# FangjinhuaWang/PatchmatchNet

Measured on AMD Instinct MI355X. Metric: depth-maps/sec at 1600x1200 N=5 src views, higher is better.
Workload: dtype f32

## Files before the change

patchmatchnet_amd/csrc/conv_f16s.hip:

```cpp
#include "pmn_common.hpp"

typedef _Float16 f16x8 __attribute__((ext_vector_type(8)));
typedef _Float16 f16x4 __attribute__((ext_vector_type(4)));
typedef float f32x4_t __attribute__((ext_vector_type(4)));
typedef float f32x2_t __attribute__((ext_vector_type(2)));
typedef _Float16 f16x2_t __attribute__((ext_vector_type(2)));

struct F16sArgs {
    int N, H, W, Ho, Wo, relu;
    int cout, ca;
    float* out_b;
};

#define PMN_F16S_LO_SCALE 2048.0f

template <int CIN, int COUT, int KS, int S, int CC, int CCP, int MT, int WPS, int DIL = 1, int OUTMODE = 0, bool SWAP = (OUTMODE == 0)>
__global__ __launch_bounds__(256, WPS) void conv_f16s_kernel(const float* __restrict__ in, const f16x8* __restrict__ wB,
                                                             const float* __restrict__ shift, float* __restrict__ out,
                                                             const F16sArgs a) {
    constexpr int NT = COUT / 16, NCB = CC / 8, CHUNKS = CIN / CC, NQ = KS * KS * NCB, KSTEPS = (NQ + 3) / 4;
    constexpr int TH = 4 * MT, TW = 16, PH = (TH - 1) * S + (KS - 1) * DIL + 1, PW = (TW - 1) * S + (KS - 1) * DIL + 1;
    constexpr int PAD = DIL * (KS / 2);
    constexpr int PLANE = PH * PW * CCP;
    constexpr int NTHR = 256;
    static_assert(!SWAP || OUTMODE == 0, "swapped operand roles (see the epilogue) serve the channels-last output");
    static_assert(CCP % 8 == 0 && CC % 8 == 0 && CIN % CC == 0, "16-byte aligned channel blocks");
    extern __shared__ float4 f16s_lds4[];
    _Float16* Phi = reinterpret_cast<_Float16*>(f16s_lds4);
    _Float16* Plo = Phi + PLANE;
    const int tid = threadIdx.x, wave = __builtin_amdgcn_readfirstlane(tid >> 6), lane = tid & 63, li = lane & 15, kb = lane >> 4;
    const int tiles_x = (a.Wo + TW - 1) / TW, tiles_y = (a.Ho + TH - 1) / TH;
    const int bt = pmn_xcd_tile(blockIdx.x, a.N * tiles_x * tiles_y);
    const int n = bt / (tiles_x * tiles_y), tr = bt - n * tiles_x * tiles_y;
    const int oy0 = (tr / tiles_x) * TH, ox0 = (tr % tiles_x) * TW;
    const int iy0 = oy0 * S - PAD, ix0 = ox0 * S - PAD;

    f32x4_t accM[MT][NT], accL[MT][NT];
#pragma unroll
    for (int t = 0; t < MT; ++t)
#pragma unroll
        for (int nt = 0; nt < NT; ++nt) {
            accM[t][nt] = f32x4_t{0.f, 0.f, 0.f, 0.f};
            accL[t][nt] = f32x4_t{0.f, 0.f, 0.f, 0.f};
        }

    const f16x8* bl = wB + lane;
    f16x8 bq[2][NT][2];
#pragma unroll
    for (int nt = 0; nt < NT; ++nt) {
        bq[0][nt][0] = bl[(size_t)((0 * NT + nt) * 2 + 0) * 64];
        bq[0][nt][1] = bl[(size_t)((0 * NT + nt) * 2 + 1) * 64];
    }

    const int q4x4 = 4 * (tid % (CC / 4)), pix_first = tid / (CC / 4);
    const int py_first = pix_first / PW, px_first = pix_first - py_first * PW, lds_first = pix_first * CCP + q4x4;

#pragma unroll 1
    for (int ch = 0; ch < CHUNKS; ++ch) {
        if (ch) __syncthreads();
        {
            constexpr int QP = CC / 4, TOT = PH * PW * QP, NL = (TOT + NTHR - 1) / NTHR, SB = 6;
            constexpr int DPIX = NTHR / QP, DY = DPIX / PW, DX = DPIX - DY * PW;
            static_assert(NTHR % QP == 0, "a step of NTHR units is a whole number of pixels");
            const float* src = in + (size_t)n * a.H * a.W * CIN + ch * CC;
            int py = py_first, px = px_first;
#pragma unroll
            for (int k0 = 0; k0 < NL; k0 += SB) {
                float4 v[SB];
#pragma unroll
                for (int k = 0; k < SB; ++k) {
                    const int gy = iy0 + py, gx = ix0 + px;
                    v[k] = make_float4(0.f, 0.f, 0.f, 0.f);
                    if (k0 + k < NL && tid < TOT - (k0 + k) * NTHR && (unsigned)gy < (unsigned)a.H && (unsigned)gx < (unsigned)a.W)
                        v[k] = *reinterpret_cast<const float4*>(src + ((unsigned)(gy * a.W + gx) * CIN + q4x4));
                    px += DX;
                    py += DY;
                    if (px >= PW) {
                        px -= PW;
                        ++py;
                    }
                }
#pragma unroll
                for (int k = 0; k < SB; ++k) {
                    if (k0 + k < NL && tid < TOT - (k0 + k) * NTHR) {
                        const f32x2_t x01 = {v[k].x, v[k].y}, x23 = {v[k].z, v[k].w};
                        const f16x2_t h01 = __builtin_convertvector(x01, f16x2_t), h23 = __builtin_convertvector(x23, f16x2_t);
                        const f16x2_t l01 = __builtin_convertvector((x01 - __builtin_convertvector(h01, f32x2_t)) * PMN_F16S_LO_SCALE, f16x2_t);
                        const f16x2_t l23 = __builtin_convertvector((x23 - __builtin_convertvector(h23, f32x2_t)) * PMN_F16S_LO_SCALE, f16x2_t);
                        const f16x4 hi = {h01[0], h01[1], h23[0], h23[1]}, lo = {l01[0], l01[1], l23[0], l23[1]};
                        *reinterpret_cast<f16x4*>(Phi + lds_first + (k0 + k) * DPIX * CCP) = hi;
                        *reinterpret_cast<f16x4*>(Plo + lds_first + (k0 + k) * DPIX * CCP) = lo;
                    }
                }
            }
        }
        __syncthreads();

#pragma unroll
        for (int ks = 0; ks < KSTEPS; ++ks) {
            constexpr int dummy = 0;
            (void)dummy;
            const int cur = ks & 1, nxt = cur ^ 1;
            {
                const int step = ch * KSTEPS + ks + 1;
                const int lim = CHUNKS * KSTEPS - 1;
                const int sidx = step < lim ? step : lim;
#pragma unroll
                for (int nt = 0; nt < NT; ++nt) {
                    bq[nxt][nt][0] = bl[(size_t)((sidx * NT + nt) * 2 + 0) * 64];
                    bq[nxt][nt][1] = bl[(size_t)((sidx * NT + nt) * 2 + 1) * 64];
                }
            }
            int q = 4 * ks + kb;
            if (4 * ks + 3 >= NQ) q = q < NQ - 1 ? q : NQ - 1;
            const int tap = q / NCB, cb = q - tap * NCB;
            const int dy = tap / KS, dx = tap - dy * KS;
            const _Float16* pa = Phi + ((wave * MT * S + dy * DIL) * PW + li * S + dx * DIL) * CCP + cb * 8;
            f16x8 ah[MT], al[MT];
#pragma unroll
            for (int t = 0; t < MT; ++t) {
                ah[t] = *reinterpret_cast<const f16x8*>(pa + t * S * PW * CCP);
                al[t] = *reinterpret_cast<const f16x8*>(pa + t * S * PW * CCP + PLANE);
            }
#pragma unroll
            for (int t = 0; t < MT; ++t)
#pragma unroll
                for (int nt = 0; nt < NT; ++nt)
                    accM[t][nt] = SWAP ? __builtin_amdgcn_mfma_f32_16x16x32_f16(bq[cur][nt][0], ah[t], accM[t][nt], 0, 0, 0)
                                       : __builtin_amdgcn_mfma_f32_16x16x32_f16(ah[t], bq[cur][nt][0], accM[t][nt], 0, 0, 0);
#pragma unroll
            for (int t = 0; t < MT; ++t)
#pragma unroll
                for (int nt = 0; nt < NT; ++nt)
                    accL[t][nt] = SWAP ? __builtin_amdgcn_mfma_f32_16x16x32_f16(bq[cur][nt][1], ah[t], accL[t][nt], 0, 0, 0)
                                       : __builtin_amdgcn_mfma_f32_16x16x32_f16(ah[t], bq[cur][nt][1], accL[t][nt], 0, 0, 0);
#pragma unroll
            for (int t = 0; t < MT; ++t)
#pragma unroll
                for (int nt = 0; nt < NT; ++nt)
                    accL[t][nt] = SWAP ? __builtin_amdgcn_mfma_f32_16x16x32_f16(bq[cur][nt][0], al[t], accL[t][nt], 0, 0, 0)
                                       : __builtin_amdgcn_mfma_f32_16x16x32_f16(al[t], bq[cur][nt][0], accL[t][nt], 0, 0, 0);
            __builtin_amdgcn_sched_barrier(0);
        }
        if (KSTEPS & 1) {
#pragma unroll
            for (int nt = 0; nt < NT; ++nt) {
                bq[0][nt][0] = bq[1][nt][0];
                bq[0][nt][1] = bq[1][nt][1];
            }
        }
    }

    if constexpr (SWAP) {
        const int ox = ox0 + li, oyw = oy0 + wave * MT;
        if (ox < a.Wo) {
            float* po = out + (((size_t)n * a.Ho + oyw) * a.Wo + ox) * COUT + 4 * kb;
            const size_t rs = (size_t)a.Wo * COUT;
            f32x4_t sh[NT];
#pragma unroll
            for (int nt = 0; nt < NT; ++nt) sh[nt] = *reinterpret_cast<const f32x4_t*>(shift + 16 * nt + 4 * kb);
#pragma unroll
            for (int t = 0; t < MT; ++t) {
                if (oyw + t < a.Ho) {
#pragma unroll
                    for (int nt = 0; nt < NT; ++nt) {
                        f32x4_t v = accM[t][nt] + accL[t][nt] * (1.0f / PMN_F16S_LO_SCALE) + sh[nt];
                        if (a.relu) v = __builtin_elementwise_max(v, f32x4_t{0.f, 0.f, 0.f, 0.f});
                        *reinterpret_cast<f32x4_t*>(po + t * rs + 16 * nt) = v;
                    }
                }
            }
        }
        return;
    }
#pragma unroll
    for (int nt = 0; nt < NT; ++nt) {
        const int c = nt * 16 + li;
        const float sh = shift[c];
#pragma unroll
        for (int t = 0; t < MT; ++t) {
            const int oy = oy0 + wave * MT + t;
            float v[4];
#pragma unroll
            for (int r = 0; r < 4; ++r) {
                v[r] = accM[t][nt][r] + accL[t][nt][r] * (1.0f / PMN_F16S_LO_SCALE) + sh;
                if (a.relu) v[r] = fmaxf(v[r], 0.0f);
            }
            if constexpr (OUTMODE == 0) {
#pragma unroll
                for (int r = 0; r < 4; ++r) {
                    const int ox = ox0 + 4 * kb + r;
                    if (oy < a.Ho && ox < a.Wo) out[(((size_t)n * a.Ho + oy) * a.Wo + ox) * COUT + c] = v[r];
                }
            } else {
                if (c < a.cout && oy < a.Ho) {
                    const bool first = c < a.ca;
                    float* dst = first ? out : a.out_b;
                    const int cx = first ? c : c - a.ca, nc = first ? a.ca : a.cout - a.ca;
                    if constexpr (OUTMODE == 1) {
                        float* row = dst + (((size_t)n * nc + cx) * a.Ho + oy) * a.Wo;
                        const int ox = ox0 + 4 * kb;
                        if ((a.Wo & 3) == 0 && ox + 3 < a.Wo) {
                            *reinterpret_cast<float4*>(row + ox) = make_float4(v[0], v[1], v[2], v[3]);
                        } else {
#pragma unroll
                            for (int r = 0; r < 4; ++r)
                                if (ox + r < a.Wo) row[ox + r] = v[r];
                        }
                    } else {
#pragma unroll
                        for (int r = 0; r < 4; ++r) {
                            const int ox = ox0 + 4 * kb + r;
                            if (ox < a.Wo) dst[(((size_t)n * a.Ho + oy) * a.Wo + ox) * nc + cx] = v[r];
                        }
                    }
                }
            }
        }
    }
}

template <int CIN, int COUT, int KS, int S, int CC, int CCP, int MT, int WPS, int DIL = 1, int OUTMODE = 0, bool SWAP = (OUTMODE == 0)>
static int launch_f16s(const float* in, const void* w, const float* shift, float* out, F16sArgs a, hipStream_t st) {
    constexpr int TH = 4 * MT, PH = (TH - 1) * S + (KS - 1) * DIL + 1, PW = 15 * S + (KS - 1) * DIL + 1;
    const size_t lds = (size_t)2 * PH * PW * CCP * sizeof(_Float16);
    auto kern = conv_f16s_kernel<CIN, COUT, KS, S, CC, CCP, MT, WPS, DIL, OUTMODE, SWAP>;
    if ((size_t)a.H * a.W * CIN >= ((size_t)1 << 30)) return PMN_ERR_SHAPE;
    if (lds > 48 * 1024 && pmn_raise_dynamic_lds(reinterpret_cast<const void*>(kern), lds) != PMN_OK) return PMN_ERR_LAUNCH;
    const int blocks = a.N * ((a.Wo + 15) / 16) * ((a.Ho + TH - 1) / TH);
    PMN_LAUNCH(kern, dim3(blocks), dim3(256), lds, st, in, reinterpret_cast<const f16x8*>(w), shift, out, a);
    PMN_CHECK_LAUNCH();
    return PMN_OK;
}

extern "C" int pmn_conv2d_f16s(const float* in, const void* weights, const float* shift, float* out, int N, int H, int W, int cin,
                               int cout, int k, int stride, int relu, void* stream) {
    if (!in || !weights || !shift || !out || N < 1 || H < 1 || W < 1) return PMN_ERR_ARG;
    F16sArgs a;
    a.N = N; a.H = H; a.W = W; a.relu = relu;
    a.cout = cout; a.ca = cout; a.out_b = nullptr;
    a.Ho = (H - 1) / (stride > 0 ? stride : 1) + 1;
    a.Wo = (W - 1) / (stride > 0 ? stride : 1) + 1;
    hipStream_t st = (hipStream_t)stream;
    if (k == 3 && stride == 1 && cin == 16 && cout == 16) return launch_f16s<16, 16, 3, 1, 16, 16, 4, 4>(in, weights, shift, out, a, st);
    if (k == 3 && stride == 1 && cin == 32 && cout == 32) return launch_f16s<32, 32, 3, 1, 16, 16, 2, 4, 1, 0, false>(in, weights, shift, out, a, st);
    if (k == 3 && stride == 1 && cin == 64 && cout == 64) return launch_f16s<64, 64, 3, 1, 16, 16, 2, 3>(in, weights, shift, out, a, st);
    if (k == 5 && stride == 2 && cin == 8 && cout == 16) return launch_f16s<8, 16, 5, 2, 8, 8, 2, 4>(in, weights, shift, out, a, st);
    if (k == 5 && stride == 2 && cin == 16 && cout == 32) return launch_f16s<16, 32, 5, 2, 8, 8, 2, 4, 1, 0, false>(in, weights, shift, out, a, st);
    if (k == 5 && stride == 2 && cin == 32 && cout == 64) return launch_f16s<32, 64, 5, 2, 16, 24, 2, 2>(in, weights, shift, out, a, st);
    return PMN_ERR_SHAPE;
}


template <int WPS>
__global__ __launch_bounds__(256, WPS) void conv_f16s_pair16_kernel(const float* __restrict__ in, const f16x8* __restrict__ wA,
                                                                   const float* __restrict__ shiftA, const f16x8* __restrict__ wBq,
                                                                   const float* __restrict__ shiftB, float* __restrict__ out,
                                                                   const F16sArgs a) {
    constexpr int C = 16, CCP = 16, NCB = 2, NQ = 18, KSTEPS = 5, TO = 14, RA = 16, PI = 18;
    constexpr int PLANE = PI * PI * CCP;
    extern __shared__ float4 f16s_pair_lds4[];
    _Float16* Phi = reinterpret_cast<_Float16*>(f16s_pair_lds4);
    _Float16* Plo = Phi + PLANE;
    const int tid = threadIdx.x, wave = __builtin_amdgcn_readfirstlane(tid >> 6), lane = tid & 63, li = lane & 15, kb = lane >> 4;
    const int tiles_x = (a.W + TO - 1) / TO, tiles_y = (a.H + TO - 1) / TO;
    const int bt = pmn_xcd_tile(blockIdx.x, a.N * tiles_x * tiles_y);
    const int n = bt / (tiles_x * tiles_y), tr = bt - n * tiles_x * tiles_y;
    const int oy0 = (tr / tiles_x) * TO, ox0 = (tr % tiles_x) * TO;

    {
        constexpr int QP = C / 4, TOT = PI * PI * QP, NL = (TOT + 255) / 256;
        const float* src = in + (size_t)n * a.H * a.W * C;
        float4 v[NL];
#pragma unroll
        for (int k = 0; k < NL; ++k) {
            const int idx = tid + k * 256, pix = idx / QP, q = idx - pix * QP;
            const int py = pix / PI, px = pix - py * PI, gy = oy0 - 2 + py, gx = ox0 - 2 + px;
            v[k] = make_float4(0.f, 0.f, 0.f, 0.f);
            if (idx < TOT && (unsigned)gy < (unsigned)a.H && (unsigned)gx < (unsigned)a.W)
                v[k] = *reinterpret_cast<const float4*>(src + ((unsigned)(gy * a.W + gx) * C + 4 * q));
        }
#pragma unroll
        for (int k = 0; k < NL; ++k) {
            const int idx = tid + k * 256, pix = idx / QP, q = idx - pix * QP;
            if (idx < TOT) {
                const f32x2_t x01 = {v[k].x, v[k].y}, x23 = {v[k].z, v[k].w};
                const f16x2_t h01 = __builtin_convertvector(x01, f16x2_t), h23 = __builtin_convertvector(x23, f16x2_t);
                const f16x2_t l01 = __builtin_convertvector((x01 - __builtin_convertvector(h01, f32x2_t)) * PMN_F16S_LO_SCALE, f16x2_t);
                const f16x2_t l23 = __builtin_convertvector((x23 - __builtin_convertvector(h23, f32x2_t)) * PMN_F16S_LO_SCALE, f16x2_t);
                const f16x4 hi = {h01[0], h01[1], h23[0], h23[1]}, lo = {l01[0], l01[1], l23[0], l23[1]};
                *reinterpret_cast<f16x4*>(Phi + pix * CCP + 4 * q) = hi;
                *reinterpret_cast<f16x4*>(Plo + pix * CCP + 4 * q) = lo;
            }
        }
    }
    __syncthreads();

    f32x4_t accM[4], accL[4];
    auto layer = [&](const f16x8* __restrict__ wq, const int pitch) {
        const f16x8* bl = wq + lane;
        f16x8 bq[2][2];
        bq[0][0] = bl[0];
        bq[0][1] = bl[64];
#pragma unroll
        for (int t = 0; t < 4; ++t) {
            accM[t] = f32x4_t{0.f, 0.f, 0.f, 0.f};
            accL[t] = f32x4_t{0.f, 0.f, 0.f, 0.f};
        }
#pragma unroll
        for (int ks = 0; ks < KSTEPS; ++ks) {
            const int cur = ks & 1, nxt = cur ^ 1;
            const int sidx = ks + 1 < KSTEPS ? ks + 1 : KSTEPS - 1;
            bq[nxt][0] = bl[(size_t)(sidx * 2 + 0) * 64];
            bq[nxt][1] = bl[(size_t)(sidx * 2 + 1) * 64];
            int q = 4 * ks + kb;
            if (4 * ks + 3 >= NQ) q = q < NQ - 1 ? q : NQ - 1;
            const int tap = q / NCB, cb = q - tap * NCB;
            const int dy = tap / 3, dx = tap - dy * 3;
            const _Float16* pa = Phi + ((wave * 4 + dy) * pitch + li + dx) * CCP + cb * 8;
            f16x8 ah[4], al[4];
#pragma unroll
            for (int t = 0; t < 4; ++t) {
                ah[t] = *reinterpret_cast<const f16x8*>(pa + t * pitch * CCP);
                al[t] = *reinterpret_cast<const f16x8*>(pa + t * pitch * CCP + PLANE);
            }
#pragma unroll
            for (int t = 0; t < 4; ++t) accM[t] = __builtin_amdgcn_mfma_f32_16x16x32_f16(bq[cur][0], ah[t], accM[t], 0, 0, 0);
#pragma unroll
            for (int t = 0; t < 4; ++t) accL[t] = __builtin_amdgcn_mfma_f32_16x16x32_f16(bq[cur][1], ah[t], accL[t], 0, 0, 0);
#pragma unroll
            for (int t = 0; t < 4; ++t) accL[t] = __builtin_amdgcn_mfma_f32_16x16x32_f16(bq[cur][0], al[t], accL[t], 0, 0, 0);
            __builtin_amdgcn_sched_barrier(0);
        }
    };

    layer(wA, PI);
    f16x4 rh[4], rl[4];
    {
        const f32x4_t sh = *reinterpret_cast<const f32x4_t*>(shiftA + 4 * kb);
        const int gx = ox0 - 1 + li;
#pragma unroll
        for (int t = 0; t < 4; ++t) {
            const int gy = oy0 - 1 + wave * 4 + t;
            f32x4_t v = accM[t] + accL[t] * (1.0f / PMN_F16S_LO_SCALE) + sh;
            if (a.relu) v = __builtin_elementwise_max(v, f32x4_t{0.f, 0.f, 0.f, 0.f});
            if (!((unsigned)gy < (unsigned)a.H && (unsigned)gx < (unsigned)a.W)) v = f32x4_t{0.f, 0.f, 0.f, 0.f};
            const f32x2_t x01 = {v[0], v[1]}, x23 = {v[2], v[3]};
            const f16x2_t h01 = __builtin_convertvector(x01, f16x2_t), h23 = __builtin_convertvector(x23, f16x2_t);
            const f16x2_t l01 = __builtin_convertvector((x01 - __builtin_convertvector(h01, f32x2_t)) * PMN_F16S_LO_SCALE, f16x2_t);
            const f16x2_t l23 = __builtin_convertvector((x23 - __builtin_convertvector(h23, f32x2_t)) * PMN_F16S_LO_SCALE, f16x2_t);
            rh[t] = f16x4{h01[0], h01[1], h23[0], h23[1]};
            rl[t] = f16x4{l01[0], l01[1], l23[0], l23[1]};
        }
    }
    __syncthreads();
#pragma unroll
    for (int t = 0; t < 4; ++t) {
        const int pix = (wave * 4 + t) * RA + li;
        *reinterpret_cast<f16x4*>(Phi + pix * CCP + 4 * kb) = rh[t];
        *reinterpret_cast<f16x4*>(Plo + pix * CCP + 4 * kb) = rl[t];
    }
    __syncthreads();

    layer(wBq, RA);
    {
        const int ox = ox0 + li;
        if (li < TO && ox < a.W) {
            const f32x4_t sh = *reinterpret_cast<const f32x4_t*>(shiftB + 4 * kb);
#pragma unroll
            for (int t = 0; t < 4; ++t) {
                const int r = wave * 4 + t, oy = oy0 + r;
                if (r < TO && oy < a.H) {
                    f32x4_t v = accM[t] + accL[t] * (1.0f / PMN_F16S_LO_SCALE) + sh;
                    if (a.relu) v = __builtin_elementwise_max(v, f32x4_t{0.f, 0.f, 0.f, 0.f});
                    *reinterpret_cast<f32x4_t*>(out + (((size_t)n * a.H + oy) * a.W + ox) * C + 4 * kb) = v;
                }
            }
        }
    }
}

extern "C" int pmn_conv2d_f16s_pair(const float* in, const void* weights_a, const float* shift_a, const void* weights_b,
                                    const float* shift_b, float* out, int N, int H, int W, int channels, int relu, void* stream) {
    if (!in || !weights_a || !shift_a || !weights_b || !shift_b || !out || N < 1 || H < 1 || W < 1) return PMN_ERR_ARG;
    if (channels != 16) return PMN_ERR_SHAPE;
    if ((size_t)H * W * 16 >= ((size_t)1 << 30)) return PMN_ERR_SHAPE;
    F16sArgs a;
    a.N = N; a.H = H; a.W = W; a.Ho = H; a.Wo = W; a.relu = relu;
    a.cout = 16; a.ca = 16; a.out_b = nullptr;
    const size_t lds = (size_t)2 * 18 * 18 * 16 * sizeof(_Float16);
    const int blocks = N * ((W + 13) / 14) * ((H + 13) / 14);
    PMN_LAUNCH(conv_f16s_pair16_kernel<4>, dim3(blocks), dim3(256), lds, (hipStream_t)stream, in, reinterpret_cast<const f16x8*>(weights_a),
               shift_a, reinterpret_cast<const f16x8*>(weights_b), shift_b, out, a);
    PMN_CHECK_LAUNCH();
    return PMN_OK;
}


template <int CIN, int DIL, int MT, int WPS>
static int dispatch_heads(const float* in, const void* w, const float* shift, float* out_a, int coutp, F16sArgs a, hipStream_t st) {
    if (coutp == 32) return launch_f16s<CIN, 32, 3, 1, 16, 16, MT, WPS, DIL, 1>(in, w, shift, out_a, a, st);
    if (coutp == 48) return launch_f16s<CIN, 48, 3, 1, 16, 16, MT, WPS, DIL, 1>(in, w, shift, out_a, a, st);
    if (coutp == 64) return launch_f16s<CIN, 64, 3, 1, 16, 16, MT, (WPS > 3 ? 3 : WPS), DIL, 1>(in, w, shift, out_a, a, st);
    return PMN_ERR_SHAPE;
}

extern "C" int pmn_offset_heads_f16s(const float* in, const void* weights, const float* shift, float* out_a, float* out_b, int N, int H,
                                     int W, int cin, int cout, int ca, int dil, void* stream) {
    if (!in || !weights || !shift || !out_a || N < 1 || H < 1 || W < 1 || cout < 1 || ca < 1 || ca > cout) return PMN_ERR_ARG;
    if (ca < cout && !out_b) return PMN_ERR_ARG;
    F16sArgs a;
    a.N = N; a.H = H; a.W = W; a.Ho = H; a.Wo = W; a.relu = 0;
    a.cout = cout; a.ca = ca; a.out_b = out_b;
    const int coutp = (cout + 15) / 16 * 16;
    hipStream_t st = (hipStream_t)stream;
    if (cin == 64 && dil == 2) return dispatch_heads<64, 2, 2, 3>(in, weights, shift, out_a, coutp, a, st);
    if (cin == 32 && dil == 4) return dispatch_heads<32, 4, 2, 4>(in, weights, shift, out_a, coutp, a, st);
    if (cin == 16 && dil == 6) return dispatch_heads<16, 6, 2, 4>(in, weights, shift, out_a, coutp, a, st);
    return PMN_ERR_SHAPE;
}

#ifndef PMN_STEM_TH
#define PMN_STEM_TH 32
#endif
template <bool VEC4, int TH>
__global__ __launch_bounds__(256, 4) void stem_f16s_kernel(const float* __restrict__ img, const float* __restrict__ w0,
                                                          const float* __restrict__ s0, const f16x8* __restrict__ w1A,
                                                          const float* __restrict__ s1, float* __restrict__ out, const int N,
                                                          const int H, const int W, const float* const* __restrict__ img_tab,
                                                          const int BV) {
    constexpr int TS = 16, IW = TH + 4, XS = 24, MW = TS + 2, MRP = 18, MROWS = TH + 2, NTHR = 256;
    static_assert(TH % 16 == 0, "a wave owns TH / 4 rows, four at a time");
    __shared__ float4 xin4[3 * IW * (XS / 4)];
    __shared__ float4 mid4[2 * MROWS * MRP];
    float* xin = reinterpret_cast<float*>(xin4);
    _Float16* midh = reinterpret_cast<_Float16*>(mid4);
    _Float16* midl = midh + MROWS * MRP * 8;
    typedef const float __attribute__((address_space(4))) cfloat;
    const cfloat* cw0 = (const cfloat*)w0;
    const cfloat* cs0 = (const cfloat*)s0;
    const int tid = threadIdx.x, wave = __builtin_amdgcn_readfirstlane(tid >> 6), lane = tid & 63, li = lane & 15, kb = lane >> 4;
    const int tiles_x = (W + TS - 1) / TS, tiles_y = (H + TH - 1) / TH;
    const int bt = pmn_xcd_tile(blockIdx.x, N * tiles_x * tiles_y);
    const int n = bt / (tiles_x * tiles_y), tr = bt - n * tiles_x * tiles_y;
    const int oy0 = (tr / tiles_x) * TH, ox0 = (tr % tiles_x) * TS;
    if (img_tab) img = img_tab[n / BV] + (ptrdiff_t)((n % BV) - n) * 3 * H * W;

    f16x8 wa[3][2];
#pragma unroll
    for (int ks = 0; ks < 3; ++ks) {
        wa[ks][0] = w1A[(ks * 2 + 0) * 64 + lane];
        wa[ks][1] = w1A[(ks * 2 + 1) * 64 + lane];
    }
    if constexpr (VEC4) {
        constexpr int NU = (3 * IW + 31) / 32;
        float4 v[NU];
        const int j = tid & 7, gx = ox0 - 4 + 4 * j;
#pragma unroll
        for (int u = 0; u < NU; ++u) {
            const int R = (tid >> 3) + 32 * u;
            const int c = (R >= IW) + (R >= 2 * IW), r = R - IW * c, gy = oy0 - 2 + r;
            v[u] = make_float4(0.f, 0.f, 0.f, 0.f);
            if (j < 6 && R < 3 * IW && (unsigned)gy < (unsigned)H && (unsigned)gx < (unsigned)W)
                v[u] = *reinterpret_cast<const float4*>(img + (((size_t)n * 3 + c) * H + gy) * W + gx);
        }
#pragma unroll
        for (int u = 0; u < NU; ++u) {
            const int R = (tid >> 3) + 32 * u;
            if (j < 6 && R < 3 * IW) xin4[R * (XS / 4) + j] = v[u];
        }
    } else {
        constexpr int NU = (3 * IW + 7) / 8;
        float v[NU];
        const int q = tid & 31, gx = ox0 - 4 + q;
#pragma unroll
        for (int u = 0; u < NU; ++u) {
            const int R = (tid >> 5) + 8 * u;
            const int c = (R >= IW) + (R >= 2 * IW), r = R - IW * c, gy = oy0 - 2 + r;
            v[u] = 0.0f;
            if (q < XS && R < 3 * IW && (unsigned)gy < (unsigned)H && (unsigned)gx < (unsigned)W)
                v[u] = img[(((size_t)n * 3 + c) * H + gy) * W + gx];
        }
#pragma unroll
        for (int u = 0; u < NU; ++u) {
            const int R = (tid >> 5) + 8 * u;
            if (q < XS && R < 3 * IW) xin[R * XS + q] = v[u];
        }
    }
    __syncthreads();
    for (int m = tid; m < MW * MROWS; m += NTHR) {
        const int r = m / MW, q = m - r * MW;
        const int gy = oy0 - 1 + r, gx = ox0 - 1 + q;
        f16x8 hi = {0, 0, 0, 0, 0, 0, 0, 0}, lo = {0, 0, 0, 0, 0, 0, 0, 0};
        if ((unsigned)gy < (unsigned)H && (unsigned)gx < (unsigned)W) {
            float acc[8];
#pragma unroll
            for (int c = 0; c < 8; ++c) acc[c] = 0.0f;
            const float* xp = xin + r * XS + q + 2;
#pragma unroll 1
            for (int ky = 0; ky < 3; ++ky) {
                const cfloat* wq = cw0 + __builtin_amdgcn_readfirstlane(ky * 72);
#pragma unroll
                for (int kx = 0; kx < 3; ++kx)
#pragma unroll
                    for (int ci = 0; ci < 3; ++ci) {
                        const float v = xp[(ci * IW + ky) * XS + kx];
#pragma unroll
                        for (int c = 0; c < 8; ++c) acc[c] = fmaf(v, wq[(kx * 3 + ci) * 8 + c], acc[c]);
                    }
            }
#pragma unroll
            for (int c = 0; c < 8; c += 2) {
                const f32x2_t x = {fmaxf(acc[c] + cs0[c], 0.0f), fmaxf(acc[c + 1] + cs0[c + 1], 0.0f)};
                const f16x2_t h = __builtin_convertvector(x, f16x2_t);
                const f32x2_t d = (x - __builtin_convertvector(h, f32x2_t)) * PMN_F16S_LO_SCALE;
                const f16x2_t l = __builtin_convertvector(d, f16x2_t);
                hi[c] = h[0];
                hi[c + 1] = h[1];
                lo[c] = l[0];
                lo[c + 1] = l[1];
            }
        }
        *reinterpret_cast<f16x8*>(midh + (r * MRP + q) * 8) = hi;
        *reinterpret_cast<f16x8*>(midl + (r * MRP + q) * 8) = lo;
    }
    __syncthreads();
#pragma unroll 1
    for (int rg = 0; rg < TH / 16; ++rg) {
    const int wrow = wave * (TH / 4) + 4 * rg;
    f32x4_t accM[4], accL[4];
#pragma unroll
    for (int t = 0; t < 4; ++t) {
        accM[t] = f32x4_t{0.f, 0.f, 0.f, 0.f};
        accL[t] = f32x4_t{0.f, 0.f, 0.f, 0.f};
    }
#pragma unroll
    for (int ks = 0; ks < 3; ++ks) {
        int q = 4 * ks + kb;
        q = q < 8 ? q : 8;
        const int dy = q / 3, dx = q - dy * 3;
        const _Float16* pb = midh + ((wrow + dy) * MRP + li + dx) * 8;
        f16x8 bh[4], blo[4];
#pragma unroll
        for (int t = 0; t < 4; ++t) {
            bh[t] = *reinterpret_cast<const f16x8*>(pb + t * MRP * 8);
            blo[t] = *reinterpret_cast<const f16x8*>(pb + t * MRP * 8 + MROWS * MRP * 8);
        }
#pragma unroll
        for (int t = 0; t < 4; ++t) accM[t] = __builtin_amdgcn_mfma_f32_16x16x32_f16(wa[ks][0], bh[t], accM[t], 0, 0, 0);
#pragma unroll
        for (int t = 0; t < 4; ++t) accL[t] = __builtin_amdgcn_mfma_f32_16x16x32_f16(wa[ks][0], blo[t], accL[t], 0, 0, 0);
#pragma unroll
        for (int t = 0; t < 4; ++t) accL[t] = __builtin_amdgcn_mfma_f32_16x16x32_f16(wa[ks][1], bh[t], accL[t], 0, 0, 0);
    }
    const int ox = ox0 + li, oyw = oy0 + wrow;
    if (kb < 2 && ox < W) {
        const f32x4_t sh = *reinterpret_cast<const f32x4_t*>(s1 + 4 * kb);
        float* po = out + (((size_t)n * H + oyw) * W + ox) * 8 + 4 * kb;
        const size_t rs = (size_t)W * 8;
#pragma unroll
        for (int t = 0; t < 4; ++t) {
            if (oyw + t < H) {
                f32x4_t v = accM[t] + accL[t] * (1.0f / PMN_F16S_LO_SCALE) + sh;
                v = __builtin_elementwise_max(v, f32x4_t{0.f, 0.f, 0.f, 0.f});
                *reinterpret_cast<f32x4_t*>(po + t * rs) = v;
            }
        }
    }
    }
}

extern "C" int pmn_stem_f16s(const float* img, const float* w0, const float* s0, const void* w1a, const float* s1, float* out,
                             int N, int H, int W, void* stream) {
    if (!img || !w0 || !s0 || !w1a || !s1 || !out || N < 1 || H < 1 || W < 1) return PMN_ERR_ARG;
    constexpr int TS = 16, TH = PMN_STEM_TH;
    const int blocks = N * ((W + TS - 1) / TS) * ((H + TH - 1) / TH);
    if (W % 4 == 0 && (reinterpret_cast<uintptr_t>(img) & 15) == 0)
        PMN_LAUNCH((stem_f16s_kernel<true, PMN_STEM_TH>), dim3(blocks), dim3(256), 0, (hipStream_t)stream, img, w0, s0,
                           reinterpret_cast<const f16x8*>(w1a), s1, out, N, H, W, nullptr, 1);
    else
        PMN_LAUNCH((stem_f16s_kernel<false, PMN_STEM_TH>), dim3(blocks), dim3(256), 0, (hipStream_t)stream, img, w0, s0,
                           reinterpret_cast<const f16x8*>(w1a), s1, out, N, H, W, nullptr, 1);
    PMN_CHECK_LAUNCH();
    return PMN_OK;
}

extern "C" int pmn_stem_f16s_views(const float* const* img_table, int views, const float* w0, const float* s0, const void* w1a,
                                   const float* s1, float* out, int B, int H, int W, void* stream) {
    if (!img_table || !w0 || !s0 || !w1a || !s1 || !out || views < 1 || B < 1 || H < 1 || W < 1) return PMN_ERR_ARG;
    constexpr int TS = 16, TH = PMN_STEM_TH;
    const int N = views * B;
    const int blocks = N * ((W + TS - 1) / TS) * ((H + TH - 1) / TH);
    if (W % 4 == 0)
        PMN_LAUNCH((stem_f16s_kernel<true, PMN_STEM_TH>), dim3(blocks), dim3(256), 0, (hipStream_t)stream, nullptr, w0, s0,
                           reinterpret_cast<const f16x8*>(w1a), s1, out, N, H, W, img_table, B);
    else
        PMN_LAUNCH((stem_f16s_kernel<false, PMN_STEM_TH>), dim3(blocks), dim3(256), 0, (hipStream_t)stream, nullptr, w0, s0,
                           reinterpret_cast<const f16x8*>(w1a), s1, out, N, H, W, img_table, B);
    PMN_CHECK_LAUNCH();
    return PMN_OK;
}
```

Before: 388.5.

## Split f16s conv waves across output-channel tiles for wide-COUT layers

```diff
diff --git a/patchmatchnet_amd/csrc/conv_f16s.hip b/patchmatchnet_amd/csrc/conv_f16s.hip
--- a/patchmatchnet_amd/csrc/conv_f16s.hip
+++ b/patchmatchnet_amd/csrc/conv_f16s.hip
@@ -14,11 +14,19 @@
 
 #define PMN_F16S_LO_SCALE 2048.0f
 
+template <int COUT, int KS, int OUTMODE>
+constexpr int f16s_waves_n() {
+    return OUTMODE == 0 && (COUT == 64 || (COUT == 32 && KS == 3)) ? 2 : 1;
+}
+
 template <int CIN, int COUT, int KS, int S, int CC, int CCP, int MT, int WPS, int DIL = 1, int OUTMODE = 0, bool SWAP = (OUTMODE == 0)>
 __global__ __launch_bounds__(256, WPS) void conv_f16s_kernel(const float* __restrict__ in, const f16x8* __restrict__ wB,
                                                              const float* __restrict__ shift, float* __restrict__ out,
                                                              const F16sArgs a) {
+    constexpr int WN = f16s_waves_n<COUT, KS, OUTMODE>();
     constexpr int NT = COUT / 16, NCB = CC / 8, CHUNKS = CIN / CC, NQ = KS * KS * NCB, KSTEPS = (NQ + 3) / 4;
+    constexpr int MTW = MT * WN, NTW = NT / WN;
+    static_assert((WN == 1 || WN == 2) && NT % WN == 0, "waves along N: 1, or 2 with an even number of N-tiles");
     constexpr int TH = 4 * MT, TW = 16, PH = (TH - 1) * S + (KS - 1) * DIL + 1, PW = (TW - 1) * S + (KS - 1) * DIL + 1;
     constexpr int PAD = DIL * (KS / 2);
     constexpr int PLANE = PH * PW * CCP;
@@ -34,20 +42,21 @@
     const int n = bt / (tiles_x * tiles_y), tr = bt - n * tiles_x * tiles_y;
     const int oy0 = (tr / tiles_x) * TH, ox0 = (tr % tiles_x) * TW;
     const int iy0 = oy0 * S - PAD, ix0 = ox0 * S - PAD;
-
-    f32x4_t accM[MT][NT], accL[MT][NT];
-#pragma unroll
-    for (int t = 0; t < MT; ++t)
-#pragma unroll
-        for (int nt = 0; nt < NT; ++nt) {
+    const int nt0 = WN == 1 ? 0 : (wave % WN) * NTW;
+
+    f32x4_t accM[MTW][NTW], accL[MTW][NTW];
+#pragma unroll
+    for (int t = 0; t < MTW; ++t)
+#pragma unroll
+        for (int nt = 0; nt < NTW; ++nt) {
             accM[t][nt] = f32x4_t{0.f, 0.f, 0.f, 0.f};
             accL[t][nt] = f32x4_t{0.f, 0.f, 0.f, 0.f};
         }
 
-    const f16x8* bl = wB + lane;
-    f16x8 bq[2][NT][2];
-#pragma unroll
-    for (int nt = 0; nt < NT; ++nt) {
+    const f16x8* bl = wB + nt0 * 2 * 64 + lane;
+    f16x8 bq[2][NTW][2];
+#pragma unroll
+    for (int nt = 0; nt < NTW; ++nt) {
         bq[0][nt][0] = bl[(size_t)((0 * NT + nt) * 2 + 0) * 64];
         bq[0][nt][1] = bl[(size_t)((0 * NT + nt) * 2 + 1) * 64];
     }
@@ -106,7 +115,7 @@
                 const int lim = CHUNKS * KSTEPS - 1;
                 const int sidx = step < lim ? step : lim;
 #pragma unroll
-                for (int nt = 0; nt < NT; ++nt) {
+                for (int nt = 0; nt < NTW; ++nt) {
                     bq[nxt][nt][0] = bl[(size_t)((sidx * NT + nt) * 2 + 0) * 64];
                     bq[nxt][nt][1] = bl[(size_t)((sidx * NT + nt) * 2 + 1) * 64];
                 }
@@ -115,36 +124,36 @@
             if (4 * ks + 3 >= NQ) q = q < NQ - 1 ? q : NQ - 1;
             const int tap = q / NCB, cb = q - tap * NCB;
             const int dy = tap / KS, dx = tap - dy * KS;
-            const _Float16* pa = Phi + ((wave * MT * S + dy * DIL) * PW + li * S + dx * DIL) * CCP + cb * 8;
-            f16x8 ah[MT], al[MT];
-#pragma unroll
-            for (int t = 0; t < MT; ++t) {
+            const _Float16* pa = Phi + (((wave / WN) * MTW * S + dy * DIL) * PW + li * S + dx * DIL) * CCP + cb * 8;
+            f16x8 ah[MTW], al[MTW];
+#pragma unroll
+            for (int t = 0; t < MTW; ++t) {
                 ah[t] = *reinterpret_cast<const f16x8*>(pa + t * S * PW * CCP);
                 al[t] = *reinterpret_cast<const f16x8*>(pa + t * S * PW * CCP + PLANE);
             }
 #pragma unroll
-            for (int t = 0; t < MT; ++t)
-#pragma unroll
-                for (int nt = 0; nt < NT; ++nt)
+            for (int t = 0; t < MTW; ++t)
+#pragma unroll
+                for (int nt = 0; nt < NTW; ++nt)
                     accM[t][nt] = SWAP ? __builtin_amdgcn_mfma_f32_16x16x32_f16(bq[cur][nt][0], ah[t], accM[t][nt], 0, 0, 0)
                                        : __builtin_amdgcn_mfma_f32_16x16x32_f16(ah[t], bq[cur][nt][0], accM[t][nt], 0, 0, 0);
 #pragma unroll
-            for (int t = 0; t < MT; ++t)
-#pragma unroll
-                for (int nt = 0; nt < NT; ++nt)
+            for (int t = 0; t < MTW; ++t)
+#pragma unroll
+                for (int nt = 0; nt < NTW; ++nt)
                     accL[t][nt] = SWAP ? __builtin_amdgcn_mfma_f32_16x16x32_f16(bq[cur][nt][1], ah[t], accL[t][nt], 0, 0, 0)
                                        : __builtin_amdgcn_mfma_f32_16x16x32_f16(ah[t], bq[cur][nt][1], accL[t][nt], 0, 0, 0);
 #pragma unroll
-            for (int t = 0; t < MT; ++t)
-#pragma unroll
-                for (int nt = 0; nt < NT; ++nt)
+            for (int t = 0; t < MTW; ++t)
+#pragma unroll
+                for (int nt = 0; nt < NTW; ++nt)
                     accL[t][nt] = SWAP ? __builtin_amdgcn_mfma_f32_16x16x32_f16(bq[cur][nt][0], al[t], accL[t][nt], 0, 0, 0)
                                        : __builtin_amdgcn_mfma_f32_16x16x32_f16(al[t], bq[cur][nt][0], accL[t][nt], 0, 0, 0);
             __builtin_amdgcn_sched_barrier(0);
         }
         if (KSTEPS & 1) {
 #pragma unroll
-            for (int nt = 0; nt < NT; ++nt) {
+            for (int nt = 0; nt < NTW; ++nt) {
                 bq[0][nt][0] = bq[1][nt][0];
                 bq[0][nt][1] = bq[1][nt][1];
             }
@@ -152,18 +161,18 @@
     }
 
     if constexpr (SWAP) {
-        const int ox = ox0 + li, oyw = oy0 + wave * MT;
+        const int ox = ox0 + li, oyw = oy0 + (wave / WN) * MTW;
         if (ox < a.Wo) {
-            float* po = out + (((size_t)n * a.Ho + oyw) * a.Wo + ox) * COUT + 4 * kb;
+            float* po = out + (((size_t)n * a.Ho + oyw) * a.Wo + ox) * COUT + 16 * nt0 + 4 * kb;
             const size_t rs = (size_t)a.Wo * COUT;
-            f32x4_t sh[NT];
-#pragma unroll
-            for (int nt = 0; nt < NT; ++nt) sh[nt] = *reinterpret_cast<const f32x4_t*>(shift + 16 * nt + 4 * kb);
-#pragma unroll
-            for (int t = 0; t < MT; ++t) {
+            f32x4_t sh[NTW];
+#pragma unroll
+            for (int nt = 0; nt < NTW; ++nt) sh[nt] = *reinterpret_cast<const f32x4_t*>(shift + 16 * (nt0 + nt) + 4 * kb);
+#pragma unroll
+            for (int t = 0; t < MTW; ++t) {
                 if (oyw + t < a.Ho) {
 #pragma unroll
-                    for (int nt = 0; nt < NT; ++nt) {
+                    for (int nt = 0; nt < NTW; ++nt) {
                         f32x4_t v = accM[t][nt] + accL[t][nt] * (1.0f / PMN_F16S_LO_SCALE) + sh[nt];
                         if (a.relu) v = __builtin_elementwise_max(v, f32x4_t{0.f, 0.f, 0.f, 0.f});
                         *reinterpret_cast<f32x4_t*>(po + t * rs + 16 * nt) = v;
@@ -174,12 +183,12 @@
         return;
     }
 #pragma unroll
-    for (int nt = 0; nt < NT; ++nt) {
-        const int c = nt * 16 + li;
+    for (int nt = 0; nt < NTW; ++nt) {
+        const int c = (nt0 + nt) * 16 + li;
         const float sh = shift[c];
 #pragma unroll
-        for (int t = 0; t < MT; ++t) {
-            const int oy = oy0 + wave * MT + t;
+        for (int t = 0; t < MTW; ++t) {
+            const int oy = oy0 + (wave / WN) * MTW + t;
             float v[4];
 #pragma unroll
             for (int r = 0; r < 4; ++r) {
```

After: 386.8. About the same (-0.4%).
